# GPUPeople/spECK

Measured on AMD Instinct MI355X. Metric: SpGEMM GFLOP/s (2*flops_intermediate/s), A*A, higher is better.
Workload: dtype f64; 1 GPU; scircuit-like A*A (SURVEY 8d stand-in); rows=170998, nnzA=965730, products=8470902, nnzC=5291656, parallelism=single

## Files before the change

speck_amd/csrc/launch.hpp:

```cpp
#pragma once
#include <hip/hip_ext.h>

#include "chain.hpp"
#include "device_common.hpp"

namespace speck {

u32 analysis_blocks(u32 m);
void set_analysis_wide_rows(u32 avg_len);
u32 scan_tiles(u32 m);

constexpr u32 kListRegions = (((u32)SYM_CLASSES > (u32)NUM_CLASSES ? (u32)SYM_CLASSES : (u32)NUM_CLASSES) + 1u) / 2u;
__host__ __device__ inline size_t class_list_records(u32 m) { return size_t(kListRegions) * (m ? m : 1u); }
template <typename Rec>
__host__ __device__ __forceinline__ Rec* class_rec_at(Rec* lists, u32 m, u32 cls, u32 i)
{
    return two_sided_at(lists, m, cls, i);
}

void launch_analysis(hipStream_t s, const u32* a_ro, const u32* a_col, const u32* b_ro, const u32* b_col, u32 m, u64 nnz_a,
                     u32* row_ops, u32* row_max_ops, u32* row_col_min, u32* row_col_max, u8* sym_cls, u32* counts,
                     RowRec* sym_recs, DeviceStats* st, const ClassifyParams& cp, uint2* b_sl, const Chain& chain,
                     u64* nf_off = nullptr, u64 expect_nf = ~0ull, u32 b_rows = ~0u,
                     u32* a_ro_copy = nullptr ,
// ... 100 lines not shown
    const u32* nf_pred_off;
    u32* nf_direct_col;
    void* nf_direct_val;
    uint2* w_sl;
    u32 xcd_aware;
    const u32* off_src;
    u32* off_dst;
    u32 off_n;
    u32 verify_counts;
    u32 verify_numeric;
    u32 sliced;
};

#ifdef __HIPCC__
__device__ __forceinline__ void store_row_count(const RowWork& w, u32* __restrict__ counts, u32 row, u32 cnt)
{
    counts[row] = cnt;
    if (w.verify_counts && cnt != w.nf_pred_off[row + 1] - w.nf_pred_off[row])
        const_cast<DeviceStats*>(w.st)->capacity_miss = 1;
}
#endif

struct ClassGrid {
    u32 first[13];
    u32 cnt[12];
};
constexpr u32 kNoCount = 0xFFFFFFFFu;
constexpr u32 kSymLightMask = (1u << SYM_BM1) | (1u << SYM_B4K) | (1u << SYM_W1K) | (1u << SYM_W256) | (1u << SYM_G16) |
                              (1u << SYM_G8) | (1u << SYM_W128) | (1u << SYM_R32) | (1u << SYM_R64);
constexpr u32 kNumLightMask = (1u << NUM_D1) | (1u << NUM_B2K) | (1u << NUM_W512) | (1u << NUM_W256) | (1u << NUM_W128) |
                              (1u << NUM_G16) | (1u << NUM_G8) | (1u << NUM_DIRECT) | (1u << NUM_R32) | (1u << NUM_R64);
constexpr u32 kNumEscMask = (1u << NUM_G8) | (1u << NUM_G16) | (1u << NUM_R32) | (1u << NUM_R64);
constexpr u32 kSymEscMask = (1u << SYM_G8) | (1u << SYM_G16) | (1u << SYM_R32) | (1u << SYM_R64);

void launch_symbolic_light(hipStream_t s, const u32* counts_hint, u32 mask, const u32* a_ro,
                           const uint2* b_sl, const u32* b_col, const RowWork& w,
                           u32* counts, int cu_count, bool exact = false, u32 fused_vsize = 0,
                           const void* a_val = nullptr, const void* b_val = nullptr, hipEvent_t e0 = nullptr,
                           hipEvent_t e1 = nullptr);
template <typename T>
void launch_numeric_light(hipStream_t s, const u32* counts_hint, u32 mask, const CsrView<T>& A,
                          const CsrView<T>& B, const RowWork& w, u32* c_col, T* c_val, int cu_count,
                          bool exact = false, hipEvent_t e0 = nullptr, hipEvent_t e1 = nullptr);

void launch_symbolic(hipStream_t s, int cls, u32 count, const u32* a_ro, const uint2* b_sl,
                     const u32* b_col, const RowWork& w, u32* counts, int cu_count);

template <typename T>
void launch_numeric_first(hipStream_t s, u32 count, const CsrView<T>& A, const CsrView<T>& B, const RowWork& w,
                          u32* counts, int cu_count, u32 wcols, hipEvent_t e0 = nullptr, hipEvent_t e1 = nullptr);

void note_launch_status(hipError_t e, const char* what);
int take_launch_error();
#define SPECK_LAUNCH(kernel_, ...)                                          \
    do {                                                                    \
        hipLaunchKernelGGL(kernel_, __VA_ARGS__);                           \
        ::speck::note_launch_status(hipGetLastError(), #kernel_);           \
    } while (0)
#define SPECK_LAUNCH_TIMED(kernel_, grid_, block_, lds_, stream_, e0_, e1_, ...)                            \
    do {                                                                                                   \
        if (e0_) hipExtLaunchKernelGGL(kernel_, grid_, block_, lds_, stream_, e0_, e1_, 0, __VA_ARGS__);   \
        else hipLaunchKernelGGL(kernel_, grid_, block_, lds_, stream_, __VA_ARGS__);                       \
        ::speck::note_launch_status(hipGetLastError(), #kernel_);                                          \
    } while (0)

template <typename T>
void launch_numeric(hipStream_t s, int cls, u32 count, const CsrView<T>& A, const CsrView<T>& B,
                    const RowWork& w, u32* c_col, T* c_val, int cu_count);

template <typename T>
void launch_walk(hipStream_t s, const WalkArgs& args, const ProductSrc<T>& src, const Chain& chain, hipEvent_t e0 = nullptr,
                 hipEvent_t e1 = nullptr);

u32 grid_for(u32 count, u32 lds, int threads, int cu_count, u32 rows_per_block);
void set_grid_rounds(u32 block_classes, u32 subwave_classes);
void set_b8k_full_first(u32 mask);
// ... 8 lines not shown
```

speck_amd/csrc/numeric.hip:

```cpp
#include <algorithm>
#include <type_traits>

#include "chain3.hpp"
#include "device_common.hpp"
#include "launch.hpp"
#include "row_groups.hpp"
#include "esc_rows.hpp"
#include "esc_wide.hpp"

namespace speck {

template <typename T, int THREADS>
constexpr u32 num_direct_lds()
{
    return THREADS * (12u + (u32)sizeof(T)) + (THREADS / 64 + 2 + win_words<Block<THREADS>>() + 3) / 4 * 16;
}

template <typename T, int THREADS>
__device__ __forceinline__ void num_direct_body(unsigned char* smem, const ProductSrc<T>& src, const RowWork& w,
                                                u32* __restrict__ c_col, T* __restrict__ c_val, u32 bidx,
                                                u32 nblk, u32 hint = kNoCount)
{
    using G = Block<THREADS>;
    const G g;
// ... 1103 lines not shown
            else
                emit_bitmap_sorted<G, T, CAP, kW256W1, CAP, false, true>(g, keys, vals, S, scan_scratch, cap_row, cmin, cmax, base,
                                                                         a.c_col, static_cast<T*>(a.c_val), NUM_W256, cnt);
        }
    }
}

template <typename T>
void launch_walk_hash(hipStream_t s, const WalkHashArgs& args, const ProductSrc<T>& src, const Chain3& chain, hipEvent_t e0,
                      hipEvent_t e1)
{
    const u32 groups = (args.m + kWalkHashRows - 1) / kWalkHashRows;
    const u32 lds = kWalkHashRows * num_group_lds<SubWave<32>, T, kNumW256Cap, 256>();
    const WalkHashArgs& a = args;
    const u32 grid = groups;
    SPECK_LAUNCH_TIMED((walk_hash_kernel<T>), dim3(grid), dim3(256), lds, s, e0, e1, src, a, chain);
}
template void launch_walk_hash<double>(hipStream_t, const WalkHashArgs&, const ProductSrc<double>&, const Chain3&, hipEvent_t, hipEvent_t);
template void launch_walk_hash<float>(hipStream_t, const WalkHashArgs&, const ProductSrc<float>&, const Chain3&, hipEvent_t, hipEvent_t);

template <typename T>
__global__ __launch_bounds__(256) void num_tiny_kernel(ProductSrc<T> src, const u32* a_ro, RowWork w,
                                                       u32* __restrict__ c_col, T* __restrict__ c_val,
                                                       ClassGrid cg)
{
    SPECK_POISON();
    extern __shared__ __attribute__((aligned(16))) unsigned char smem[];
    src.rebase(a_ro);
    const u32 b = blockIdx.x;
    if (b < cg.first[5])
        num_escw_body<T, 64, 256>(smem, src, w, c_col, c_val, NUM_R64, b - cg.first[4], cg.first[5] - cg.first[4], cg.cnt[4]);
    else if (b < cg.first[6])
        num_escw_body<T, 32, 256>(smem, src, w, c_col, c_val, NUM_R32, b - cg.first[5], cg.first[6] - cg.first[5], cg.cnt[5]);
    else if (b < cg.first[7])
        num_hash_body<SubWave<32>, T, kNumW128Cap, 0, kNumW128MaxNnz, SORT_RANK, 256>(
            smem, src, w, c_col, c_val, NUM_W128, b - cg.first[6], cg.first[7] - cg.first[6], cg.cnt[6]);
    else if (b < cg.first[8])
        num_esc_body<T, 16, 256>(smem, src, w, c_col, c_val, NUM_G16, b - cg.first[7], cg.first[8] - cg.first[7], cg.cnt[7]);
    else if (b < cg.first[9])
        num_esc_body<T, 8, 256>(smem, src, w, c_col, c_val, NUM_G8, b - cg.first[8], cg.first[9] - cg.first[8], cg.cnt[8]);
    else
        num_direct_body<T, 256>(smem, src, w, c_col, c_val, b - cg.first[9], cg.first[10] - cg.first[9], cg.cnt[9]);
}

constexpr u32 kGParts = 16;
constexpr u32 kGMaxBuckets = 2048;
constexpr u32 kGMaxCells = 4096;
constexpr int kGWalkThreads = 256;

__global__ __launch_bounds__(1024) void num_spill_plan_kernel(RowWork w, int cls)
{
    SPECK_POISON();
    __shared__ u32 s_scan[1024 / 64 + 2];
    __shared__ u64 s_run_p;
    __shared__ u32 s_run_b, s_run_f;
    if (block_void(w.st->capacity_miss)) return;
    const u32 count = min(w.st->num.count[cls], w.m);
    if (threadIdx.x == 0) {
        s_run_p = 0;
        s_run_b = 0;
        s_run_f = 0;
    }
    __syncthreads();
    for (u32 i0 = 0; i0 < count; i0 += 1024) {
        const u32 i = i0 + threadIdx.x;
        u32 ops = 0, nb = 0, nf = 0, shift = 0, unit = 1;
        if (i < count) {
            const RowRec rec = *class_rec_at(w.recs, w.m, cls, i);
            ops = rec.ops;
            const u32 range_m1 = rec.cmax - rec.cmin;
            nb = (ops + kGBucketTarget - 1) / kGBucketTarget;
            nb = nb < 1u ? 1u : (nb > kGMaxBuckets ? kGMaxBuckets : nb);
            unit = (ops + nb - 1) / nb;
            const u32 cells = min(kGMaxCells, kGCellsPerBucket * nb);
            while ((range_m1 >> shift) + 1u > cells) ++shift;
// ... 380 lines not shown

u32 numeric_lds_bytes(int cls, u32 vsize)
{
    return vsize == 8 ? numeric_lds_bytes_t<double>(cls) : numeric_lds_bytes_t<float>(cls);
}

template <typename K>
static void set_dyn_lds(K kernel, u32 bytes)
{
    if (bytes > 48 * 1024)
        note_launch_status(hipFuncSetAttribute(reinterpret_cast<const void*>(kernel),
                                               hipFuncAttributeMaxDynamicSharedMemorySize, (int)bytes),
                           "hipFuncSetAttribute(MaxDynamicSharedMemorySize)");
}

template <class G, typename T, u32 CAP, u32 W1, u32 NMAX, int MODE, int THREADS, u32 NLO = 0, bool VERIFY = false>
static void launch_num_hash(hipStream_t s, int cls, u32 count, const ProductSrc<T>& A, const u32* B,
                            const RowWork& w, u32* c_col, T* c_val, int cu_count)
{
    auto k = num_hash_kernel<G, T, CAP, W1, NMAX, MODE, THREADS, NLO, VERIFY>;
    const u32 lds = (THREADS / G::SIZE) * num_group_lds<G, T, CAP, THREADS>();
    set_dyn_lds(k, lds);
    SPECK_LAUNCH(k, dim3(grid_for(count, lds, THREADS, cu_count, THREADS / G::SIZE)),
                       dim3(THREADS), lds, s, A, B, w, c_col, c_val, cls);
}

static u32 g_b8k_full_first = 1;
void set_b8k_full_first(u32 mask) { g_b8k_full_first = mask; }
static u32 g_spill_big_grid = 256;
void set_spill_big_grid(u32 blocks) { g_spill_big_grid = blocks ? blocks : 256u; }

template <typename T>
void launch_numeric_light(hipStream_t s, const u32* counts_hint, u32 mask, const CsrView<T>& Av,
                          const CsrView<T>& Bv, const RowWork& w, u32* c_col, T* c_val, int cu_count, bool exact,
                          hipEvent_t e0, hipEvent_t e1)
{
    constexpr int NS = 10;
    static const int slots[NS] = {NUM_D1, NUM_B2K, NUM_W512, NUM_W256, NUM_R64, NUM_R32, NUM_W128, NUM_G16, NUM_G8, NUM_DIRECT};
    static const u32 rows_per_block[NS] = {1, 1, 4, 8, 4, 8, 8, 16, 32, 256};
    bool tiny_only = true;
    for (int k = 0; k < 4; ++k)
        if ((mask >> slots[k] & 1u) && counts_hint[slots[k]]) tiny_only = false;
    if (w.verify_numeric || w.off_n) tiny_only = false;
    u32 lds = 0;
    for (int k = 0; k < NS; ++k)
        if (mask >> slots[k] & 1u) lds = std::max(lds, numeric_lds_bytes_t<T>(slots[k]));
    ClassGrid cg{};
    for (int k = 0; k < NS; ++k) {
        const bool on = (mask >> slots[k] & 1u) && counts_hint[slots[k]];
        cg.first[k + 1] = cg.first[k] + (on ? grid_for(counts_hint[slots[k]], lds, 256, cu_count, rows_per_block[k]) : 0u);
        cg.cnt[k] = exact ? counts_hint[slots[k]] : kNoCount;
    }
    cg.first[NS + 1] = cg.first[NS];
    if (!tiny_only && w.off_n) cg.first[NS + 1] += std::min<u32>((w.off_n + 2047u) / 2048u, 512u);
    if (cg.first[NS + 1] == 0) {
        if (e0) (void)hipEventRecord(e0, s), (void)hipEventRecord(e1, s);
        return;
    }
    const ProductSrc<T> src{w.b_sl, Av.data, Bv.col_ids, Bv.data, w.w_sl};
    bool with_esc = false;
    for (int k = 0; k < NS; ++k)
        if ((kNumEscMask >> slots[k] & 1u) && cg.first[k + 1] != cg.first[k]) with_esc = true;
    if (w.verify_numeric)
        SPECK_LAUNCH_TIMED((num_light_kernel<T, false, true>), dim3(cg.first[NS + 1]), dim3(256), lds, s, e0, e1, src,
                           Av.row_offsets, w, c_col, c_val, cg);
    else if (!tiny_only && with_esc)
        SPECK_LAUNCH_TIMED((num_light_kernel<T, true>), dim3(cg.first[NS + 1]), dim3(256), lds, s, e0, e1, src, Av.row_offsets, w,
                           c_col, c_val, cg);
    else if (!tiny_only)
        SPECK_LAUNCH_TIMED((num_light_kernel<T, false>), dim3(cg.first[NS + 1]), dim3(256), lds, s, e0, e1, src, Av.row_offsets, w,
                           c_col, c_val, cg);
    else
        SPECK_LAUNCH_TIMED((num_tiny_kernel<T>), dim3(cg.first[NS]), dim3(256), lds, s, e0, e1, src, Av.row_offsets, w,
                           c_col, c_val, cg);
}
// ... 149 lines not shown
            auto ks = num_spill_scatter_kernel<T>;
            SPECK_LAUNCH(ks, dim3(rows, kGParts), dim3(kGWalkThreads), (num_spill_walk_lds<T, true>()), s,
                               A, B, w, cls);
            auto kr_small = num_spill_reduce_kernel<T, kNumB2KCap, kB2KW1, 256, 0, kNumB2KMaxNnz, false>;
            SPECK_LAUNCH(kr_small, dim3(rows, 32), dim3(256), (num_spill_reduce_lds<T, kNumB2KCap, 256>()), s, w,
                               cls);
            auto kr_big = num_spill_reduce_kernel<T, kNumB8KCap, kB8KW1, 512, kNumB2KMaxNnz, kNumB8KCap * 85 / 100, true>;
            set_dyn_lds(kr_big, lds);
            SPECK_LAUNCH(kr_big, dim3(g_spill_big_grid), dim3(512), lds, s, w, cls);
            SPECK_LAUNCH((num_spill_copy_kernel<T>), dim3(rows, 32), dim3(256), 0, s, w, c_col, c_val, cls);
            break;
        }
    }
}

}
#ifdef SPECK_PHASE_CLOCKS
extern "C" int speck_debug_phase_clocks(unsigned long long* out)
{
    constexpr int n = speck::kMaxClasses * 16;
    static unsigned long long all[speck::kPhaseSlots * n];
    if (hipMemcpyFromSymbol(all, HIP_SYMBOL(speck::g_phase_clk), sizeof(all)) != hipSuccess) return 3;
    for (int i = 0; i < n; ++i) out[i] = 0;
    for (int s = 0; s < speck::kPhaseSlots; ++s)
        for (int i = 0; i < n; ++i) out[i] += all[s * n + i];
    for (auto& x : all) x = 0;
    return hipMemcpyToSymbol(HIP_SYMBOL(speck::g_phase_clk), all, sizeof(all)) == hipSuccess ? 0 : 3;
}
#endif
namespace speck {

template void launch_numeric_light<double>(hipStream_t, const u32*, u32, const CsrView<double>&,
                                           const CsrView<double>&, const RowWork&, u32*, double*, int, bool,
                                           hipEvent_t, hipEvent_t);
template void launch_numeric_light<float>(hipStream_t, const u32*, u32, const CsrView<float>&,
                                          const CsrView<float>&, const RowWork&, u32*, float*, int, bool, hipEvent_t,
                                          hipEvent_t);
template void launch_numeric_first<double>(hipStream_t, u32, const CsrView<double>&, const CsrView<double>&,
                                           const RowWork&, u32*, int, u32, hipEvent_t, hipEvent_t);
template void launch_numeric_first<float>(hipStream_t, u32, const CsrView<float>&, const CsrView<float>&,
                                          const RowWork&, u32*, int, u32, hipEvent_t, hipEvent_t);
template void launch_numeric<double>(hipStream_t, int, u32, const CsrView<double>&,
                                     const CsrView<double>&, const RowWork&, u32*, double*, int);
template void launch_numeric<float>(hipStream_t, int, u32, const CsrView<float>&,
                                    const CsrView<float>&, const RowWork&, u32*, float*, int);

}
```

speck_amd/csrc/pipeline.hip:

```cpp
#include <hip/hip_runtime.h>

#include <algorithm>
#include <chrono>
#include <cstdio>
#include <cstdlib>
#include <cstring>
#include <functional>
#include <string>
#include <vector>

#include "../../include/speck_c_api.h"
#include "chain3.hpp"
#include "host_common.hpp"
#include "launch.hpp"
#include "row_groups.hpp"
#include "masked.hpp"
#include "select.hpp"
#include "add.hpp"
#include "reduce.hpp"
#include "scale.hpp"
#include "sort_rows.hpp"

using namespace speck;

// ... 67 lines not shown
    u32* d_ticket = nullptr;
    u32* h_ticket = nullptr;
    u32* h_ticket_dev = nullptr;
    u32 ticket_expected = 0;
    bool spin_wait = true;
    void* chain_buf = nullptr;
    u64 chain_launches = 0;
    u32 chain_fault = ~0u;
    u64* d_bytes = nullptr;
    ClassifyParams cp{};
    int profile_kernels = 0;
    std::vector<hipEvent_t> kev;
    std::vector<hipStream_t> aux;
    std::vector<hipEvent_t> aux_done;
    hipEvent_t fork = nullptr;
    hipEvent_t vgate = nullptr;
    u64 validate_after_nnz = 1ull << 25;
    bool eager_speculate = true;
    bool spec_valid = false;
    bool eager_through = true;
    const u32* through_gate = nullptr;
    u32 through_ticket = 0;
    hipEvent_t vdone = nullptr;
    u64 through_hits = 0, through_misses = 0;
    u64 spec_rows_a = 0, spec_rows_b = 0;
    int eager_spec_hits = 0, eager_spec_misses = 0;
    const u32* stage_off_src = nullptr;
    u32* stage_off_dst = nullptr;
    u32 stage_off_n = 0;
    bool validate_inputs = true;
    bool concurrent_classes = true;
    u32 max_side_streams = 12;
    float fork_min_us = 60.f;
    u32 xcd_aware = 10;
    u32 last_sym_counts[kMaxClasses] = {}, last_num_counts[kMaxClasses] = {};

    bool reuse = true;
    bool plan_valid = false;
    CallKey plan_key;
    u32 last_sym_mask = 0, last_num_mask = 0;
    u32 last_max_row_nnz = 0;
    CallKey last_key;
    bool last_key_valid = false;
    int replays = 0, plans_made = 0, replay_misses = 0;
    void* gpool = nullptr;
    size_t gpool_bytes = 0;
    void* nfpool = nullptr;
    size_t nfpool_bytes = 0;
    u64 nf_cap_entries = 0;
    size_t nf_pool_max_bytes = 0;
    int pool_fallbacks = 0;
    Prediction pred, gpred;
    DeviceStats last_eager_stats{};
    bool pred_valid = false;
    bool nf_direct = true;
    bool capture_direct = false;
    bool esc_fused = true;
    bool capture_fused = false;
    u32* capture_c_col = nullptr;
    void* capture_c_val = nullptr;
    ReplayPlan plan{};
    bool skip_scan = true;
    bool capture_skip_scan = false;
    int num_verify = 1;
    bool capture_num_verify = false;
    u32* snap = nullptr;
// ... 305 lines not shown
        (void)hipEventSynchronize(c->individualEnd);
        (void)hipEventElapsedTime(&ms, c->individualStart, c->individualEnd);
        start();
        return ms;
    }
};

int check_inputs(const speck_dcsr* A, const speck_dcsr* B)
{
    if (!A || !B) return SPECK_ERR_INVALID;
    if (A->cols != B->rows) return SPECK_ERR_INVALID;
    if (B->cols > (1ull << 27) || A->rows > (1ull << 27)) return SPECK_ERR_DIM_LIMIT;
    if (A->rows && !A->row_offsets) return SPECK_ERR_INVALID;
    if (B->rows && !B->row_offsets) return SPECK_ERR_INVALID;
    return SPECK_OK;
}

hipEvent_t kernel_event(speck_config* c, size_t i)
{
    while (c->kev.size() <= i) {
        hipEvent_t e;
        (void)hipEventCreate(&e);
        c->kev.push_back(e);
    }
    return c->kev[i];
}

struct ClassTiming {
    int cls;
    size_t ev;
};

constexpr int kLight = -1;

template <typename LaunchFn>
int run_classes(speck_config* c, hipStream_t s, const int* order, int n_order, u32 mask, u32 light_mask,
                const u32* counts, const float* ns_per_row, size_t* ev_idx, std::vector<ClassTiming>* timing,
                int exact_cls, LaunchFn&& launch)
{
    bool forked = false;
    size_t used = 0;
    auto active = [&](int cls) { return cls == kLight ? (mask & light_mask) != 0 : (mask >> cls & 1u) != 0; };
    auto est_us = [&](int cls) -> float {
        if (!counts) return 1e9f;
        const u32 m = cls == kLight ? (mask & light_mask) : (1u << cls);
        float us = 0.f;
        for (int k = 0; k < kMaxClasses; ++k)
            if (m >> k & 1u) us += counts[k] * ns_per_row[k] * 1e-3f;
        return us;
    };
    int n_big = 0;
    for (int i = 0; i < n_order; ++i)
        if (active(order[i]) && est_us(order[i]) >= c->fork_min_us) ++n_big;
    int last_active = -1;
    for (int i = 0; i < n_order; ++i)
        if (active(order[i])) last_active = i;
    if (n_big >= 2)
        for (int i = 0; i < n_order; ++i)
            if (active(order[i]) && est_us(order[i]) >= c->fork_min_us) last_active = i;
    const size_t max_side = std::min<size_t>(c->aux.size(), c->max_side_streams);
    size_t touched = 0;
    int seq[kMaxClasses + 2];
    int n_seq = 0;
    for (int i = 0; i < n_order; ++i)
        if (active(order[i])) seq[n_seq++] = i;
    if (counts)
        std::stable_sort(seq, seq + n_seq, [&](int a, int b) { return est_us(order[a]) > est_us(order[b]); });
    auto on_side = [&](int i) {
        return c->concurrent_classes && max_side > 0 && i != last_active && n_big >= 2 && est_us(order[i]) >= c->fork_min_us;
    };
    for (int q = 0; q < n_seq && !forked; ++q)
        if (on_side(seq[q])) {
            HIP_TRY(hipEventRecord(c->fork, s));
            forked = true;
        }
    for (int q = 0; q < n_seq; ++q) {
        const int i = seq[q];
        const int cls = order[i];
        hipStream_t ks = s;
        if (on_side(i)) {
            const size_t slot = std::min(used, max_side - 1);
            ks = c->aux[slot];
            if (slot >= touched) {
                HIP_TRY(hipStreamWaitEvent(ks, c->fork, 0));
                touched = slot + 1;
            }
            ++used;
        }
        const bool timed = c->profile_kernels == 1 && timing;
        const bool exact = timed && (cls == kLight || cls == exact_cls);
        hipEvent_t e0 = timed ? kernel_event(c, *ev_idx) : nullptr, e1 = timed ? kernel_event(c, *ev_idx + 1) : nullptr;
        if (timed && !exact) (void)hipEventRecord(e0, ks);
        launch(ks, cls, exact ? e0 : nullptr, exact ? e1 : nullptr);
        if (timed) {
            if (!exact) (void)hipEventRecord(e1, ks);
            timing->push_back({cls, *ev_idx});
            *ev_idx += 2;
        }
    }
    for (size_t k = 0; k < touched; ++k) {
        HIP_TRY(hipEventRecord(c->aux_done[k], c->aux[k]));
        HIP_TRY(hipStreamWaitEvent(s, c->aux_done[k], 0));
    }
    LAUNCHES_OK();
    return SPECK_OK;
}

constexpr float kSymNsPerRow[kMaxClasses] = {0.15f, 0.6f, 3.f, 5.f, 30.f, 1000.f, 8.5f, 1000.f, 12.f, 50000.f, 0.1f, 0.4f,
                                             0.4f, 0.8f, 0.f, 0.f};
constexpr float kNumNsPerRow[kMaxClasses] = {0.1f, 0.3f, 2.f, 4.f, 12.f, 75.f, 12.f, 300.f, 1500.f, 2.5f, 1.5f, 0.2f,
                                             0.6f, 1.2f, 0.f, 0.f};
constexpr u32 kAllSym = (1u << SYM_CLASSES) - 1u;
constexpr u32 kAllNum = (1u << NUM_CLASSES) - 1u;

u32 mask_of(const u32* counts, int n)
{
    u32 m = 0;
    for (int i = 0; i < n; ++i)
        if (counts[i]) m |= 1u << i;
    return m;
}

struct Timing {
// ... 120 lines not shown
            const ProductSrc<float> src{sc.b_sl, static_cast<const float*>(A->data), B->col_ids, static_cast<const float*>(B->data), sc.w_sl};
            launch_walk<float>(s, wa, src, chain, e0, e1);
        }
        LAUNCHES_OK();
        return SPECK_OK;
    }
    if (timed) {
        tm->ev_scan = tm->ev;
        (void)hipEventRecord(kernel_event(c, tm->ev++), s);
    }
    if (c->capture_skip_scan) {
    } else {
        Chain chain;
        const int crc = next_chain(c, s, &chain);
        if (crc != SPECK_OK) return crc;
        if (c->through_gate && !c->through_ticket) {
            HIP_TRY(hipEventRecord(c->vdone, c->vstream));
            HIP_TRY(hipStreamWaitEvent(s, c->vdone, 0));
        }
        launch_scan(s, c_ro, sc.offsets, m, A->row_offsets, sc.row_ops, sc.row_col_min, sc.row_col_max,
                    classify_numeric ? sc.num_recs : nullptr, c->d_stats, cp, vsize, exact_nnz, chain, host_mirror,
                    expect_g, expect_g_rows, c->capture_direct ? c->gpred.off : nullptr, pred_off_out,
                    host_mirror ? c->d_ticket : nullptr, host_mirror ? c->h_ticket_dev : nullptr, bytes, c->through_gate,
                    c->through_ticket);
    }
    if (timed) (void)hipEventRecord(kernel_event(c, tm->ev++), s);
    LAUNCHES_OK();
    return SPECK_OK;
}

template <typename T>
int enqueue_back(speck_config* c, hipStream_t s, const speck_dcsr* A, const speck_dcsr* B,
                 const Scratch& sc, u32* c_col, T* c_val, u32 num_mask,
                 const u32* counts , Timing* tm)
{
    const u32 m = (u32)A->rows;
    CsrView<T> Av{c->capture_overlap ? sc.a_ro_copy : A->row_offsets, A->col_ids, static_cast<const T*>(A->data), m, (u32)A->cols};
    CsrView<T> Bv{B->row_offsets, B->col_ids, static_cast<const T*>(B->data), (u32)B->rows,
                  (u32)B->cols};
    RowWork w = make_work(c, sc, c->spill, m);
    w.sliced = (c->cp.slice_ops && u64(B->cols) <= kSliceMaxCols) ? 1u : 0u;
    if (w.off_n && !(num_mask & kNumLightMask)) {
        launch_copy_offsets(s, w.off_src, w.off_dst, w.off_n, c->d_stats);
        w.off_n = 0;
    }
    u32 all_m[kMaxClasses];
    for (auto& x : all_m) x = m;
    const u32* hint = counts ? counts : all_m;
    static const int order[5] = {NUM_G, NUM_D2, NUM_B8K, NUM_NFCOPY, kLight};
    return run_classes(c, s, order, 5, num_mask, kNumLightMask, counts, kNumNsPerRow, tm ? &tm->ev : nullptr,
                       tm ? &tm->num : nullptr, -100,
                       [&](hipStream_t ks, int cls, hipEvent_t e0, hipEvent_t e1) {
                           if (cls == kLight)
                               launch_numeric_light<T>(ks, hint, num_mask & kNumLightMask, Av, Bv, w, c_col, c_val, c->sm,
                                                       counts != nullptr, e0, e1);
                           else
                               launch_numeric<T>(ks, cls, hint[cls], Av, Bv, w, c_col, c_val, c->sm);
                       });
}

int wait_ticket(speck_config* c, hipStream_t s)
{
    if (c->spin_wait) {
        const u32 want = ++c->ticket_expected;
        const auto t0 = std::chrono::steady_clock::now();
        bool seen = false;
        while (!(seen = __atomic_load_n(c->h_ticket, __ATOMIC_ACQUIRE) == want)) {
            for (int i = 0; i < 64; ++i) cpu_relax();
            if (std::chrono::steady_clock::now() - t0 > kSpinBudget) break;
        }
        if (!seen) HIP_TRY(hipStreamSynchronize(s));
    } else {
        HIP_TRY(hipStreamSynchronize(s));
    }
    c->ticket_expected = __atomic_load_n(c->h_ticket, __ATOMIC_ACQUIRE);
    return SPECK_OK;
}

int read_stats(speck_config* c, hipStream_t s)
{
    if (c->spin_wait) {
        launch_done(s, c->d_ticket, c->h_ticket_dev, c->d_stats, c->h_stats_dev);
        const int rc = wait_ticket(c, s);
        if (rc != SPECK_OK) return rc;
    } else {
        HIP_TRY(hipMemcpyAsync(c->h_stats, c->d_stats, sizeof(DeviceStats), hipMemcpyDeviceToHost, s));
        HIP_TRY(hipStreamSynchronize(s));
    }
    return c->h_stats->chain_error ? chain_failed(c, s) : SPECK_OK;
}

// ... 128 lines not shown
    }
    int rc = enqueue_front(c, s, A, B, sc, (u32)sizeof(T), C->nnz, sym_mask, p.num_mask, true, tm, sym_counts, nullptr,
                           p.g_products, p.num_counts[NUM_G], 3u, p.nf_cap_entries);
    if (rc != SPECK_OK) return rc;
    if (tm) {
        tm->ev_num = tm->ev;
        (void)hipEventRecord(kernel_event(c, tm->ev++), s);
    }
    rc = enqueue_back<T>(c, s, A, B, sc, C->col_ids, static_cast<T*>(C->data), p.launch_mask, p.num_counts, tm);
    if (rc != SPECK_OK) return rc;
    if (tm) {
        *ev_num_end = tm->ev;
        (void)hipEventRecord(kernel_event(c, tm->ev++), s);
    }
    launch_done(s, c->d_ticket, c->h_ticket_dev, c->d_stats, c->h_stats_dev);
    return SPECK_OK;
}

void publish_kernel_times(speck_config* c, const Timing& tm, size_t ev_num_end)
{
    auto ms = [&](size_t a) {
        float v = 0.f;
        (void)hipEventElapsedTime(&v, c->kev[a], c->kev[a + 1]);
        return v;
    };
    (void)hipEventElapsedTime(&c->last.analysis_ms, c->kev[tm.ev_analysis], c->kev[tm.ev_analysis_end]);
    c->last.scan_ms = ms(tm.ev_scan);
    (void)hipEventElapsedTime(&c->last.sym_phase_ms, c->kev[tm.ev_analysis_end], c->kev[tm.ev_scan]);
    (void)hipEventElapsedTime(&c->last.num_phase_ms, c->kev[tm.ev_num], c->kev[ev_num_end]);
    for (const auto& ct : tm.sym) {
        if (ct.cls == kLight) c->last.sym_light_ms = ms(ct.ev);
        else c->last.sym_bin_ms[ct.cls] = ms(ct.ev);
    }
    for (const auto& ct : tm.num) {
        if (ct.cls == kLight) c->last.num_light_ms = ms(ct.ev);
        else c->last.num_bin_ms[ct.cls] = ms(ct.ev);
    }
    c->last.kernel_events_valid = 1;
}

int launch_verifier(speck_config* c, const speck_dcsr* A, const speck_dcsr* B, const Scratch& sc)
{
    __atomic_store_n(c->h_verify, 0u, __ATOMIC_RELEASE);
    c->verifier_in_flight = true;
    auto validate = [&] {
        if (c->validate_inputs)
            launch_validate_b(c->vstream, B->row_offsets, B->col_ids, (u32)B->rows, (u32)B->cols, B->nnz, c->h_verify_dev);
    };
    if (c->verify_inputs && c->snap && c->snap_for_arena) {
        launch_verify_inputs(c->vstream, A->row_offsets, sc.a_ro_copy, (u32)A->rows, A->col_ids, c->snap, A->nnz, B->row_offsets,
                             B->col_ids, (u32)B->rows, c->snap + c->snap_a_words, c->h_verify_dev);
        validate();
        launch_ticket(c->vstream, c->d_vticket, c->h_verify_dev + 16);
        LAUNCHES_OK();
        return SPECK_OK;
    }
    ClassifyParams cp = c->cp;
    cp.sym_allowed = cp.num_allowed = 0xFFFFFFFFu;
    cp.esc16 = (c->cp.esc16 && B->cols <= (1ull << 26)) ? 1u : 0u;
    cp.esc_fused = 0;
    launch_analysis(c->vstream, A->row_offsets, A->col_ids, B->row_offsets, B->col_ids, (u32)A->rows, A->nnz, sc.row_ops,
                    sc.row_max_ops, sc.row_col_min, sc.row_col_max, sc.cls_sym, sc.counts, sc.sym_recs, c->d_stats, cp,
                    sc.b_sl, Chain{nullptr, nullptr, nullptr, 0u, ~0u}, sc.nf_off, ~0ull, (u32)B->rows, sc.a_ro_copy, c->h_verify_dev, nullptr, B->nnz);
    if (c->verify_inputs && c->snap) {
        launch_snapshot_inputs(c->vstream, A->row_offsets, A->col_ids, c->snap, A->nnz, B->row_offsets, B->col_ids, (u32)B->rows,
                               c->snap + c->snap_a_words);
        c->snap_pending = true;
    }
    validate();
// ... 350 lines not shown
                validate_started = false;
            }
        }
    }
    bool through_ok = false, through_missed = false, through_front = false;
    if (!walked && c->eager_through && c->eager_speculate && c->spec_valid && c->spec_rows_a == A->rows && c->spec_rows_b == B->rows &&
        c_ready && C->nnz <= 0xFFFFFFFFull && C->nnz == c->last_eager_stats.nnz_c && c->last_num_mask && !c->last_was_walk &&
        !c->profile_kernels && !t->measureAll && c->spin_wait && !c->cp.want_bytes &&
        (!(c->last_num_mask >> NUM_G & 1u) || c->spill.plan != nullptr)) {
        u32 hints[kMaxClasses], mask = kSymLightMask;
        for (int k = 0; k < kMaxClasses; ++k) {
            hints[k] = c->last_sym_counts[k];
            if (hints[k]) mask |= 1u << k;
            if ((kSymLightMask >> k & 1u) && !hints[k]) hints[k] = 256;
        }
        struct ThroughFlags {
            speck_config* c;
            ~ThroughFlags()
            {
                c->through_gate = nullptr, c->through_ticket = 0;
                c->stage_off_src = nullptr, c->stage_off_dst = nullptr, c->stage_off_n = 0;
            }
        } through_flags{c};
        c->through_gate = c->validate_inputs ? c->h_verify_dev : nullptr;
        c->through_ticket = (c->validate_inputs && B->nnz < c->validate_after_nnz) ? c->vticket_expected + 1u : 0u;
        c->stage_off_src = sc.offsets;
        c->stage_off_dst = C->row_offsets;
        c->stage_off_n = m + 1;
        const bool has_g = (c->last_num_mask >> NUM_G & 1u) != 0;
        rc = enqueue_front(c, s, A, B, sc, (u32)sizeof(T), C->nnz, mask, c->last_num_mask, true, &tm, hints, nullptr,
                           has_g ? c->last_g_products : ~0ull, has_g ? c->last_num_counts[NUM_G] : ~0u, 3u, c->nf_cap_entries,
                           keep_pred ? c->pred.off : nullptr, true);
        if (rc != SPECK_OK) return fail(rc);
        rc = enqueue_back<T>(c, s, A, B, sc, C->col_ids, static_cast<T*>(C->data), c->last_num_mask, c->last_num_counts, &tm);
        if (rc != SPECK_OK) return fail(rc);
        rc = read_stats(c, s);
        if (rc != SPECK_OK) return fail(rc);
        if (c->h_stats->a_invalid) return fail(SPECK_ERR_INVALID);
        bool b_bad = false;
        rc = b_is_invalid(&b_bad);
        if (rc != SPECK_OK) return fail(rc);
        if (b_bad) return fail(SPECK_ERR_UNSORTED);
        through_ok = !c->h_stats->capacity_miss && !c->h_stats->nnz_overflow && c->h_stats->nnz_c == C->nnz &&
                     c->h_stats->sum_products != 0;
        ++(through_ok ? c->through_hits : c->through_misses);
        if (through_ok) {
            publish_counts(c, s);
            num_mask = mask_of(c->h_stats->num.count, NUM_CLASSES);
            c->last_g_products = c->h_stats->g_products;
            c->last.eager_speculated = 1;
            c->last.eager_through = 1;
            t->countProducts = t->loadBalanceCounting = t->globalMapsCounting = t->globalMapsNumeric = t->allocC = t->loadBalanceNumeric = 0.f;
            t->spGEMMCounting = 0.f;
            t->spGEMMNumeric = st.lap();
        } else if (!c->h_stats->front_miss && !c->h_stats->nnz_overflow) {
            HIP_TRY(hipMemsetAsync(&c->d_stats->capacity_miss, 0, sizeof(u32), s));
            c->h_stats->capacity_miss = 0;
            through_missed = through_front = true;
        } else {
            validate_started = false;
            tm = Timing{};
            through_missed = true;
        }
    }
    if (!walked && !through_ok) {
    bool speculated = through_front;
    if (through_front) c->last.eager_speculated = 1;
// ... 137 lines not shown
            return fail(SPECK_ERR_OOM);
        }
        if (C->data) (void)guarded_free(C->data);
        if (C->col_ids) (void)guarded_free(C->col_ids);
        if (C->row_offsets && C->row_offsets != c_ro) (void)guarded_free(C->row_offsets);
        c_val = nv;
        c_col = nc;
    } else if (C->row_offsets && C->row_offsets != c_ro) {
        (void)guarded_free(C->row_offsets);
    }
    C->rows = A->rows;
    C->cols = B->cols;
    C->nnz = nnz_c;
    C->data = c_val;
    C->col_ids = c_col;
    C->row_offsets = c_ro;
    own_ro = false;
    struct Unstage {
        speck_config* c;
        ~Unstage() { c->stage_off_src = nullptr, c->stage_off_dst = nullptr, c->stage_off_n = 0; }
    } unstage{c};
    c->stage_off_src = sc.offsets;
    c->stage_off_dst = c_ro;
    c->stage_off_n = m + 1;
    t->allocC = st.lap();
    t->loadBalanceNumeric = 0.f;


    c->last_g_products = c->h_stats->g_products;
    if (c->profile_kernels) {
        tm.ev_num = tm.ev;
        (void)hipEventRecord(kernel_event(c, tm.ev++), s);
    }
    rc = enqueue_back<T>(c, s, A, B, sc, c_col, static_cast<T*>(c_val), num_mask, c->h_stats->num.count, &tm);
    if (rc != SPECK_OK) return rc;
    ev_num_end = tm.ev;
    if (c->profile_kernels) (void)hipEventRecord(kernel_event(c, tm.ev++), s);
    if (c->spin_wait && !c->profile_kernels) {
        launch_done(s, c->d_ticket, c->h_ticket_dev, c->d_stats, c->h_stats_dev);
        rc = wait_ticket(c, s);
        if (rc != SPECK_OK) return rc;
    } else {
        HIP_TRY(hipStreamSynchronize(s));
    }
    t->spGEMMNumeric = st.lap();
    }
    t->sorting = 0.f;
    t->cleanup = 0.f;

    c->last_was_walk = walked;
    c->last_nf_entries = c->h_stats->nf_entries;
    c->last_sym_mask = mask_of(c->h_stats->sym.count, SYM_CLASSES);
    c->last_num_mask = num_mask;
    c->last_max_row_nnz = c->h_stats->max_row_nnz_c;
    c->last_max_row_ops = c->h_stats->max_row_ops;
    std::memcpy(c->last_sym_counts, c->h_stats->sym.count, sizeof(c->last_sym_counts));
    std::memcpy(c->last_num_counts, c->h_stats->num.count, sizeof(c->last_num_counts));
    c->last_key = make_key<T>(c, A, B, C, s);
    c->last_key_valid = true;
    c->arena_key = c->last_key;
    c->arena_key_valid = true;
    c->arena_from_replay = false;
    c->spec_valid = true;
    c->spec_rows_a = A->rows;
    c->spec_rows_b = B->rows;
    c->pred_valid = keep_pred;
    c->last_eager_stats = *c->h_stats;
// ... 239 lines not shown
        c->sort.release();
        c->masked.release();
        c->select.release();
        c->add.release();
        c->reduce.release();
        c->scale.release();
    }
    else if (n == "sort_reg_max") c->sort.reg_max = (u32)std::min<int64_t>(std::max<int64_t>(value, 0), SPECK_SORT_REG_MAX);
    else if (n == "sort_lds_max") c->sort.lds_max = (u32)std::min<int64_t>(std::max<int64_t>(value, 0), SPECK_SORT_LDS_MAX);
    else if (n == "mask_group_max") c->masked.group_max = (u32)std::min<int64_t>(std::max<int64_t>(value, 0), SPECK_MASK_GROUP_MAX);
    else if (n == "mask_lds_max") c->masked.lds_max = (u32)std::min<int64_t>(std::max<int64_t>(value, 0), SPECK_MASK_LDS_MAX);
    else if (n == "walk_debug") set_walk_debug((u32)value & 0xFFFFu, (u32)(value >> 16));
    else if (n == "verify_inputs") c->verify_inputs = value != 0, c->snap_for_arena = false, forget(false);
    else if (n == "num_verify") c->num_verify = (int)value, forget(false);
    else if (n == "skip_scan") c->skip_scan = value != 0, forget(false);
    else if (n == "overlap_analysis") c->overlap_analysis = value != 0, forget(false);
    else if (n == "esc_fused") c->esc_fused = value != 0, forget(true);
    else if (n == "nf_direct") c->nf_direct = value != 0, forget(false);
    else if (n == "sym_w128") c->cp.sym_w128 = value != 0, forget(true);
    else if (n == "sym_g8") c->cp.sym_g8 = value != 0, forget(true);
    else if (n == "esc16") c->cp.esc16 = value != 0, forget(true);
    else if (n == "slice_rows") c->cp.slice_ops = value ? kSliceMaxOps : 0u, forget(true);
    else if (n == "esc32") c->cp.esc32 = value != 0, forget(true);
    else if (n == "esc64") c->cp.esc64 = value != 0, forget(true);
    else if (n == "num_g8") c->cp.num_g8 = value != 0, forget(true);
    else if (n == "num_w256") c->cp.num_w256 = value != 0, forget(true);
    else if (n == "collect_bytes") c->cp.want_bytes = value != 0;
    else if (n == "concurrent_classes") c->concurrent_classes = value != 0;
    else if (n == "validate_inputs") c->validate_inputs = value != 0;
    else if (n == "validate_after_nnz") c->validate_after_nnz = (u64)value;
    else if (n == "spin_wait") c->spin_wait = value != 0, forget(false);
    else if (n == "fork_min_us") c->fork_min_us = (float)value, forget(false);
    else if (n == "max_side_streams") c->max_side_streams = (u32)value, forget(false);
    else if (n == "reuse" || n == "use_graph") {
        if (c->reuse != (value != 0)) forget(true);
        c->reuse = value != 0;
    }
    else if (n == "grid_rounds_block") set_grid_rounds((u32)value, 0), forget(false);
    else if (n == "grid_rounds_sub") set_grid_rounds(0, (u32)value), forget(false);
    else if (n == "spill_big_grid") set_spill_big_grid((u32)value), forget(false);
    else if (n == "scan_small_items") set_scan_small_items((int)value), forget(true);
    else if (n == "b8k_full_first") set_b8k_full_first((u32)value), forget(false);
    else if (n == "xcd_aware") c->xcd_aware = (u32)value, forget(false);
    else return SPECK_ERR_INVALID;
    return SPECK_OK;
}

int speck_config_profile_kernels(speck_config* c, int enable)
{
    if (!c) return SPECK_ERR_INVALID;
    c->profile_kernels = enable == 2 ? 2 : (enable != 0 ? 1 : 0);
    return SPECK_OK;
}

int speck_last_stats(const speck_config* c, speck_stats* out)
{
    if (!c || !out) return SPECK_ERR_INVALID;
    *out = c->last;
    out->numeric_reruns = c->replay_misses;
    out->graph_replays = c->replays;
    out->graph_captures = c->plans_made;
    out->pool_fallbacks = c->pool_fallbacks;
    out->scratch_pool_bytes = c->nfpool_bytes;
    out->walk_misses = c->walk_misses;
    return SPECK_OK;
}
// ... 153 lines not shown
```

Measured before the change: 127.0 GFLOP/s.

## Split light numeric classes into register and hash kernels, optionally on separate streams

Adds a kernel that handles only the hash-based light numeric classes, next to the existing register/ESC tiny kernel. An auto mode picks the specialised kernel when only one group has rows, which should reduce the register and LDS footprint of the light launch. An optional split_light setting, off by default, runs the two parts concurrently on a side stream. W128 is moved out of the tiny kernel, and the scheduler and per-class timing logic are reworked to handle the two parts.

```diff
diff --git a/speck_amd/csrc/launch.hpp b/speck_amd/csrc/launch.hpp
--- a/speck_amd/csrc/launch.hpp
+++ b/speck_amd/csrc/launch.hpp
@@ -156,6 +156,15 @@
                               (1u << NUM_G16) | (1u << NUM_G8) | (1u << NUM_DIRECT) | (1u << NUM_R32) | (1u << NUM_R64);
 constexpr u32 kNumEscMask = (1u << NUM_G8) | (1u << NUM_G16) | (1u << NUM_R32) | (1u << NUM_R64);
 constexpr u32 kSymEscMask = (1u << SYM_G8) | (1u << SYM_G16) | (1u << SYM_R32) | (1u << SYM_R64);
+constexpr u32 kNumRegMask = kNumEscMask | (1u << NUM_DIRECT);
+constexpr u32 kNumHashMask = kNumLightMask & ~kNumRegMask;
+inline bool light_part_rows(const u32* counts, u32 part_mask)
+{
+    for (int k = 0; k < NUM_CLASSES; ++k)
+        if ((part_mask >> k & 1u) && counts[k]) return true;
+    return false;
+}
+enum { kLightMerged = 0, kLightAuto = 1, kLightReg = 2, kLightHash = 3 };
 
 void launch_symbolic_light(hipStream_t s, const u32* counts_hint, u32 mask, const u32* a_ro,
                            const uint2* b_sl, const u32* b_col, const RowWork& w,
@@ -165,7 +174,7 @@
 template <typename T>
 void launch_numeric_light(hipStream_t s, const u32* counts_hint, u32 mask, const CsrView<T>& A,
                           const CsrView<T>& B, const RowWork& w, u32* c_col, T* c_val, int cu_count,
-                          bool exact = false, hipEvent_t e0 = nullptr, hipEvent_t e1 = nullptr);
+                          bool exact = false, hipEvent_t e0 = nullptr, hipEvent_t e1 = nullptr, int form = kLightMerged);
 
 void launch_symbolic(hipStream_t s, int cls, u32 count, const u32* a_ro, const uint2* b_sl,
                      const u32* b_col, const RowWork& w, u32* counts, int cu_count);
diff --git a/speck_amd/csrc/numeric.hip b/speck_amd/csrc/numeric.hip
--- a/speck_amd/csrc/numeric.hip
+++ b/speck_amd/csrc/numeric.hip
@@ -1159,15 +1159,43 @@
         num_escw_body<T, 64, 256>(smem, src, w, c_col, c_val, NUM_R64, b - cg.first[4], cg.first[5] - cg.first[4], cg.cnt[4]);
     else if (b < cg.first[6])
         num_escw_body<T, 32, 256>(smem, src, w, c_col, c_val, NUM_R32, b - cg.first[5], cg.first[6] - cg.first[5], cg.cnt[5]);
-    else if (b < cg.first[7])
-        num_hash_body<SubWave<32>, T, kNumW128Cap, 0, kNumW128MaxNnz, SORT_RANK, 256>(
-            smem, src, w, c_col, c_val, NUM_W128, b - cg.first[6], cg.first[7] - cg.first[6], cg.cnt[6]);
     else if (b < cg.first[8])
         num_esc_body<T, 16, 256>(smem, src, w, c_col, c_val, NUM_G16, b - cg.first[7], cg.first[8] - cg.first[7], cg.cnt[7]);
     else if (b < cg.first[9])
         num_esc_body<T, 8, 256>(smem, src, w, c_col, c_val, NUM_G8, b - cg.first[8], cg.first[9] - cg.first[8], cg.cnt[8]);
-    else
+    else if (b < cg.first[10])
         num_direct_body<T, 256>(smem, src, w, c_col, c_val, b - cg.first[9], cg.first[10] - cg.first[9], cg.cnt[9]);
+    else if (!w.st->capacity_miss)
+        for (u32 i = (b - cg.first[10]) * 256u + threadIdx.x; i < w.off_n; i += (cg.first[11] - cg.first[10]) * 256u)
+            w.off_dst[i] = w.off_src[i];
+}
+
+template <typename T>
+__global__ __launch_bounds__(256) void num_hashed_kernel(ProductSrc<T> src, const u32* a_ro, RowWork w,
+                                                         u32* __restrict__ c_col, T* __restrict__ c_val,
+                                                         ClassGrid cg)
+{
+    SPECK_POISON();
+    extern __shared__ __attribute__((aligned(16))) unsigned char smem[];
+    src.rebase(a_ro);
+    const u32 b = blockIdx.x;
+    if (b < cg.first[1])
+        num_dense_body<T, kNumD1Win, 256>(smem, src, w, c_col, c_val, NUM_D1, b - cg.first[0], cg.first[1] - cg.first[0], cg.cnt[0]);
+    else if (b < cg.first[2])
+        num_hash_body<Block<256>, T, kNumB2KCap, kB2KW1, kNumB2KMaxNnz, SORT_BITMAP, 256>(
+            smem, src, w, c_col, c_val, NUM_B2K, b - cg.first[1], cg.first[2] - cg.first[1], cg.cnt[1]);
+    else if (b < cg.first[3])
+        num_hash_body<SubWave<64>, T, kNumW512Cap, kW512W1, kNumW512MaxNnz, SORT_BITMAP, 256>(
+            smem, src, w, c_col, c_val, NUM_W512, b - cg.first[2], cg.first[3] - cg.first[2], cg.cnt[2]);
+    else if (b < cg.first[4])
+        num_hash_body<SubWave<32>, T, kNumW256Cap, kW256W1, kNumW256MaxNnz, SORT_BITMAP, 256>(
+            smem, src, w, c_col, c_val, NUM_W256, b - cg.first[3], cg.first[4] - cg.first[3], cg.cnt[3]);
+    else if (b < cg.first[7])
+        num_hash_body<SubWave<32>, T, kNumW128Cap, 0, kNumW128MaxNnz, SORT_RANK, 256>(
+            smem, src, w, c_col, c_val, NUM_W128, b - cg.first[6], cg.first[7] - cg.first[6], cg.cnt[6]);
+    else if (!w.st->capacity_miss)
+        for (u32 i = (b - cg.first[10]) * 256u + threadIdx.x; i < w.off_n; i += (cg.first[11] - cg.first[10]) * 256u)
+            w.off_dst[i] = w.off_src[i];
 }
 
 constexpr u32 kGParts = 16;
@@ -1614,15 +1642,48 @@
 
 template <typename T>
 void launch_numeric_light(hipStream_t s, const u32* counts_hint, u32 mask, const CsrView<T>& Av,
-                          const CsrView<T>& Bv, const RowWork& w, u32* c_col, T* c_val, int cu_count, bool exact,
-                          hipEvent_t e0, hipEvent_t e1)
+                          const CsrView<T>& Bv, const RowWork& w_in, u32* c_col, T* c_val, int cu_count, bool exact,
+                          hipEvent_t e0, hipEvent_t e1, int form)
 {
     constexpr int NS = 10;
     static const int slots[NS] = {NUM_D1, NUM_B2K, NUM_W512, NUM_W256, NUM_R64, NUM_R32, NUM_W128, NUM_G16, NUM_G8, NUM_DIRECT};
     static const u32 rows_per_block[NS] = {1, 1, 4, 8, 4, 8, 8, 16, 32, 256};
+    RowWork w = w_in;
+    if (form == kLightAuto) {
+        const bool reg = light_part_rows(counts_hint, mask & kNumRegMask), hash = light_part_rows(counts_hint, mask & kNumHashMask);
+        form = w.verify_numeric || (reg && hash) ? kLightMerged : (hash ? kLightHash : kLightReg);
+    } else if (form == kLightHash) {
+        w.off_n = 0;
+    }
+    if (form == kLightReg || form == kLightHash) {
+        mask &= form == kLightReg ? kNumRegMask : kNumHashMask;
+        u32 lds = 0;
+        for (int k = 0; k < NS; ++k)
+            if (mask >> slots[k] & 1u) lds = std::max(lds, numeric_lds_bytes_t<T>(slots[k]));
+        ClassGrid cg{};
+        for (int k = 0; k < NS; ++k) {
+            const bool on = (mask >> slots[k] & 1u) && counts_hint[slots[k]];
+            cg.first[k + 1] = cg.first[k] + (on ? grid_for(counts_hint[slots[k]], lds, 256, cu_count, rows_per_block[k]) : 0u);
+            cg.cnt[k] = exact ? counts_hint[slots[k]] : kNoCount;
+        }
+        cg.first[NS + 1] = cg.first[NS] + (w.off_n ? std::min<u32>((w.off_n + 2047u) / 2048u, 512u) : 0u);
+        if (cg.first[NS + 1] == 0) {
+            if (e0) (void)hipEventRecord(e0, s), (void)hipEventRecord(e1, s);
+            return;
+        }
+        const ProductSrc<T> src{w.b_sl, Av.data, Bv.col_ids, Bv.data, w.w_sl};
+        if (form == kLightReg)
+            SPECK_LAUNCH_TIMED((num_tiny_kernel<T>), dim3(cg.first[NS + 1]), dim3(256), lds, s, e0, e1, src, Av.row_offsets, w,
+                               c_col, c_val, cg);
+        else
+            SPECK_LAUNCH_TIMED((num_hashed_kernel<T>), dim3(cg.first[NS + 1]), dim3(256), lds, s, e0, e1, src, Av.row_offsets, w,
+                               c_col, c_val, cg);
+        return;
+    }
     bool tiny_only = true;
     for (int k = 0; k < 4; ++k)
         if ((mask >> slots[k] & 1u) && counts_hint[slots[k]]) tiny_only = false;
+    if ((mask >> NUM_W128 & 1u) && counts_hint[NUM_W128]) tiny_only = false;
     if (w.verify_numeric || w.off_n) tiny_only = false;
     u32 lds = 0;
     for (int k = 0; k < NS; ++k)
@@ -1838,10 +1899,10 @@
 
 template void launch_numeric_light<double>(hipStream_t, const u32*, u32, const CsrView<double>&,
                                            const CsrView<double>&, const RowWork&, u32*, double*, int, bool,
-                                           hipEvent_t, hipEvent_t);
+                                           hipEvent_t, hipEvent_t, int);
 template void launch_numeric_light<float>(hipStream_t, const u32*, u32, const CsrView<float>&,
                                           const CsrView<float>&, const RowWork&, u32*, float*, int, bool, hipEvent_t,
-                                          hipEvent_t);
+                                          hipEvent_t, int);
 template void launch_numeric_first<double>(hipStream_t, u32, const CsrView<double>&, const CsrView<double>&,
                                            const RowWork&, u32*, int, u32, hipEvent_t, hipEvent_t);
 template void launch_numeric_first<float>(hipStream_t, u32, const CsrView<float>&, const CsrView<float>&,
diff --git a/speck_amd/csrc/pipeline.hip b/speck_amd/csrc/pipeline.hip
--- a/speck_amd/csrc/pipeline.hip
+++ b/speck_amd/csrc/pipeline.hip
@@ -123,6 +123,7 @@
     bool concurrent_classes = true;
     u32 max_side_streams = 12;
     float fork_min_us = 60.f;
+    bool split_light = false;
     u32 xcd_aware = 10;
     u32 last_sym_counts[kMaxClasses] = {}, last_num_counts[kMaxClasses] = {};
 
@@ -494,43 +495,73 @@
 };
 
 constexpr int kLight = -1;
+constexpr int kHashLight = -2;
 
 template <typename LaunchFn>
 int run_classes(speck_config* c, hipStream_t s, const int* order, int n_order, u32 mask, u32 light_mask,
                 const u32* counts, const float* ns_per_row, size_t* ev_idx, std::vector<ClassTiming>* timing,
-                int exact_cls, LaunchFn&& launch)
+                int exact_cls, LaunchFn&& launch, u32 split_mask = 0, bool* split_out = nullptr)
 {
     bool forked = false;
     size_t used = 0;
-    auto active = [&](int cls) { return cls == kLight ? (mask & light_mask) != 0 : (mask >> cls & 1u) != 0; };
-    auto est_us = [&](int cls) -> float {
+    bool split = false;
+    int side_cls = -100;
+    auto light_bits = [&](int cls) -> u32 {
+        const u32 l = mask & light_mask;
+        if (!split) return cls == kLight ? l : 0u;
+        return cls == kLight ? l & ~split_mask : l & split_mask;
+    };
+    auto active = [&](int cls) { return cls < 0 ? light_bits(cls) != 0 : (mask >> cls & 1u) != 0; };
+    auto est_bits = [&](u32 m) -> float {
         if (!counts) return 1e9f;
-        const u32 m = cls == kLight ? (mask & light_mask) : (1u << cls);
         float us = 0.f;
         for (int k = 0; k < kMaxClasses; ++k)
             if (m >> k & 1u) us += counts[k] * ns_per_row[k] * 1e-3f;
         return us;
     };
-    int n_big = 0;
-    for (int i = 0; i < n_order; ++i)
-        if (active(order[i]) && est_us(order[i]) >= c->fork_min_us) ++n_big;
-    int last_active = -1;
-    for (int i = 0; i < n_order; ++i)
-        if (active(order[i])) last_active = i;
-    if (n_big >= 2)
+    auto est_us = [&](int cls) -> float { return est_bits(cls < 0 ? light_bits(cls) : (1u << cls)); };
+    auto big = [&](int i) {
+        const int cls = order[i];
+        if (!active(cls) || cls == side_cls) return false;
+        return (cls < 0 ? est_bits(mask & light_mask) : est_us(cls)) >= c->fork_min_us;
+    };
+    int n_big = 0, last_active = -1;
+    auto plan = [&] {
+        n_big = 0;
         for (int i = 0; i < n_order; ++i)
-            if (active(order[i]) && est_us(order[i]) >= c->fork_min_us) last_active = i;
+            if (big(i)) ++n_big;
+        last_active = -1;
+        for (int i = 0; i < n_order; ++i)
+            if (active(order[i]) && order[i] != side_cls) last_active = i;
+        if (n_big >= 2)
+            for (int i = 0; i < n_order; ++i)
+                if (big(i)) last_active = i;
+    };
+    plan();
     const size_t max_side = std::min<size_t>(c->aux.size(), c->max_side_streams);
     size_t touched = 0;
+    auto on_side = [&](int i) {
+        if (order[i] == side_cls) return true;
+        return c->concurrent_classes && max_side > 0 && i != last_active && n_big >= 2 && big(i);
+    };
+    if (split_mask && counts && c->concurrent_classes && max_side > 0 && light_part_rows(counts, mask & light_mask & split_mask) &&
+        light_part_rows(counts, mask & light_mask & ~split_mask)) {
+        size_t n_side = 0;
+        for (int i = 0; i < n_order; ++i)
+            if (active(order[i]) && on_side(i)) ++n_side;
+        if (n_side < max_side) {
+            split = true;
+            side_cls = est_us(kHashLight) <= est_us(kLight) ? kHashLight : kLight;
+            plan();
+        }
+    }
+    if (split_out) *split_out = split;
     int seq[kMaxClasses + 2];
     int n_seq = 0;
     for (int i = 0; i < n_order; ++i)
         if (active(order[i])) seq[n_seq++] = i;
     if (counts)
         std::stable_sort(seq, seq + n_seq, [&](int a, int b) { return est_us(order[a]) > est_us(order[b]); });
-    auto on_side = [&](int i) {
-        return c->concurrent_classes && max_side > 0 && i != last_active && n_big >= 2 && est_us(order[i]) >= c->fork_min_us;
-    };
     for (int q = 0; q < n_seq && !forked; ++q)
         if (on_side(seq[q])) {
             HIP_TRY(hipEventRecord(c->fork, s));
@@ -550,7 +581,7 @@
             ++used;
         }
         const bool timed = c->profile_kernels == 1 && timing;
-        const bool exact = timed && (cls == kLight || cls == exact_cls);
+        const bool exact = timed && (cls == kLight || cls == kHashLight || cls == exact_cls);
         hipEvent_t e0 = timed ? kernel_event(c, *ev_idx) : nullptr, e1 = timed ? kernel_event(c, *ev_idx + 1) : nullptr;
         if (timed && !exact) (void)hipEventRecord(e0, ks);
         launch(ks, cls, exact ? e0 : nullptr, exact ? e1 : nullptr);
@@ -737,7 +768,8 @@
 template <typename T>
 int enqueue_back(speck_config* c, hipStream_t s, const speck_dcsr* A, const speck_dcsr* B,
                  const Scratch& sc, u32* c_col, T* c_val, u32 num_mask,
-                 const u32* counts , Timing* tm)
+                 const u32* counts , Timing* tm,
+                 bool complete_call = false )
 {
     const u32 m = (u32)A->rows;
     CsrView<T> Av{c->capture_overlap ? sc.a_ro_copy : A->row_offsets, A->col_ids, static_cast<const T*>(A->data), m, (u32)A->cols};
@@ -752,16 +784,21 @@
     u32 all_m[kMaxClasses];
     for (auto& x : all_m) x = m;
     const u32* hint = counts ? counts : all_m;
-    static const int order[5] = {NUM_G, NUM_D2, NUM_B8K, NUM_NFCOPY, kLight};
-    return run_classes(c, s, order, 5, num_mask, kNumLightMask, counts, kNumNsPerRow, tm ? &tm->ev : nullptr,
+    const bool own_kernels = complete_call && counts && !w.verify_numeric;
+    bool split = false;
+    static const int order[6] = {NUM_G, NUM_D2, NUM_B8K, NUM_NFCOPY, kHashLight, kLight};
+    return run_classes(c, s, order, 6, num_mask, kNumLightMask, counts, kNumNsPerRow, tm ? &tm->ev : nullptr,
                        tm ? &tm->num : nullptr, -100,
                        [&](hipStream_t ks, int cls, hipEvent_t e0, hipEvent_t e1) {
-                           if (cls == kLight)
+                           if (cls == kLight || cls == kHashLight)
                                launch_numeric_light<T>(ks, hint, num_mask & kNumLightMask, Av, Bv, w, c_col, c_val, c->sm,
-                                                       counts != nullptr, e0, e1);
+                                                       counts != nullptr, e0, e1,
+                                                       cls == kHashLight ? kLightHash
+                                                                         : (split ? kLightReg : (own_kernels ? kLightAuto : kLightMerged)));
                            else
                                launch_numeric<T>(ks, cls, hint[cls], Av, Bv, w, c_col, c_val, c->sm);
-                       });
+                       },
+                       own_kernels && c->split_light ? kNumHashMask : 0u, &split);
 }
 
 int wait_ticket(speck_config* c, hipStream_t s)
@@ -956,9 +993,20 @@
         if (ct.cls == kLight) c->last.sym_light_ms = ms(ct.ev);
         else c->last.sym_bin_ms[ct.cls] = ms(ct.ev);
     }
+    size_t light[2] = {0, 0};
+    int n_light = 0;
     for (const auto& ct : tm.num) {
-        if (ct.cls == kLight) c->last.num_light_ms = ms(ct.ev);
+        if (ct.cls == kLight || ct.cls == kHashLight) light[n_light++] = ct.ev;
         else c->last.num_bin_ms[ct.cls] = ms(ct.ev);
+    }
+    if (n_light == 1) c->last.num_light_ms = ms(light[0]);
+    if (n_light == 2) {
+        float lead = 0.f, a = 0.f, b = 0.f;
+        (void)hipEventElapsedTime(&lead, c->kev[light[0]], c->kev[light[1]]);
+        const size_t first = lead >= 0.f ? light[0] : light[1];
+        (void)hipEventElapsedTime(&a, c->kev[first], c->kev[light[0] + 1]);
+        (void)hipEventElapsedTime(&b, c->kev[first], c->kev[light[1] + 1]);
+        c->last.num_light_ms = std::max(a, b);
     }
     c->last.kernel_events_valid = 1;
 }
@@ -1375,7 +1423,7 @@
                            has_g ? c->last_g_products : ~0ull, has_g ? c->last_num_counts[NUM_G] : ~0u, 3u, c->nf_cap_entries,
                            keep_pred ? c->pred.off : nullptr, true);
         if (rc != SPECK_OK) return fail(rc);
-        rc = enqueue_back<T>(c, s, A, B, sc, C->col_ids, static_cast<T*>(C->data), c->last_num_mask, c->last_num_counts, &tm);
+        rc = enqueue_back<T>(c, s, A, B, sc, C->col_ids, static_cast<T*>(C->data), c->last_num_mask, c->last_num_counts, &tm, true);
         if (rc != SPECK_OK) return fail(rc);
         rc = read_stats(c, s);
         if (rc != SPECK_OK) return fail(rc);
@@ -1579,7 +1627,7 @@
         tm.ev_num = tm.ev;
         (void)hipEventRecord(kernel_event(c, tm.ev++), s);
     }
-    rc = enqueue_back<T>(c, s, A, B, sc, c_col, static_cast<T*>(c_val), num_mask, c->h_stats->num.count, &tm);
+    rc = enqueue_back<T>(c, s, A, B, sc, c_col, static_cast<T*>(c_val), num_mask, c->h_stats->num.count, &tm, true);
     if (rc != SPECK_OK) return rc;
     ev_num_end = tm.ev;
     if (c->profile_kernels) (void)hipEventRecord(kernel_event(c, tm.ev++), s);
@@ -1885,6 +1933,7 @@
     else if (n == "spin_wait") c->spin_wait = value != 0, forget(false);
     else if (n == "fork_min_us") c->fork_min_us = (float)value, forget(false);
     else if (n == "max_side_streams") c->max_side_streams = (u32)value, forget(false);
+    else if (n == "split_light") c->split_light = value != 0, forget(false);
     else if (n == "reuse" || n == "use_graph") {
         if (c->reuse != (value != 0)) forget(true);
         c->reuse = value != 0;
```

Result: no change. 126.8 GFLOP/s (-0.1%).
